# mlpc-ucsd/BDM

Measured on AMD Instinct MI355X. Metric: sampled shapes/sec (4096 pts, 1000 DDPM steps), higher is better.
Workload: dtype f32

## Files before the change

bdm_amd/csrc/pvconv_compact.hip:

```cpp
#include <stdlib.h>

#include "../../include/bdm_hip.h"
#include "common.h"
#include "gn_rule.h"
#include "h2_split.h"
#include "se_fc.h"
#include "trilinear.h"

using namespace bdm;

typedef __attribute__((ext_vector_type(8))) _Float16 f16x8;

namespace {

__device__ __forceinline__ void all_group_stats(const double *__restrict__ partial, int bi, int G, int S, double count, float eps,
                                                float *s_mean, float *s_rstd) {
  const int tid = threadIdx.x, l = tid & 31, gq = tid >> 5, per = blockDim.x >> 5;
  for (int g0 = 0; g0 < G; g0 += per) {
    const int g = g0 + gq;
    double a = 0.0, q = 0.0;
    if (g < G) {
      const double *pp = partial + ((size_t)bi * G + g) * S * 2;
      for (int sl = l; sl < S; sl += 32) { a += pp[2 * sl]; q += pp[2 * sl + 1]; }
    }
    a = half32_sum(a); q = half32_sum(q);
    if (l == 0 && g < G) gn_mean_rstd(a, q, count, eps, s_mean[g], s_rstd[g]);
  }
  __syncthreads();
}

}

__global__ __launch_bounds__(256) void to_h2_rows_kernel(int C, int V, int G, int S, int n_rows_max, int tiles_max, int dense_in,
                                                         const float *__restrict__ x, const int *__restrict__ dil_list,
                                                         const int *__restrict__ tile_start, const float *__restrict__ bias,
                                                         const double *__restrict__ partial, const float *__restrict__ gamma,
                                                         const float *__restrict__ beta, float eps, int act, float act_scale,
                                                         uint4 *__restrict__ rows_h2, uint4 *__restrict__ const_h2,
                                                         float *__restrict__ const_f32, unsigned *__restrict__ saturated) {
  __shared__ float s_mean[64], s_rstd[64];
  __shared__ float s_a[256], s_b[256];
  const int bi = blockIdx.y, tid = threadIdx.x, lane = tid & 63;
  const int C8 = (C + 7) / 8;
  const int nd = tile_start[((size_t)bi * tiles_max + tiles_max - 1) * 16 + 1];
  constexpr int RB = 512;
  if ((int)blockIdx.x * RB >= nd && blockIdx.x != 0) return;
  const int cg = C / G;
  const float g_pre = tid < C ? gamma[tid] : 0.f, b_pre = tid < C ? beta[tid] : 0.f;
  const int per_pass = blockDim.x / C8;
  const int c8 = tid % C8, rl = tid / C8;
  const int nch = min(8, C - c8 * 8);
  const bool vec = (C & 3) == 0 && nch == 8;
  auto load_row = [&](int j, float (&in)[8]) {
    if (dense_in) {
      const int v = dil_list[(size_t)bi * n_rows_max + j];
      const float *xb = x + ((size_t)bi * C + c8 * 8) * V + v;
#pragma unroll
      for (int u = 0; u < 8; ++u) in[u] = xb[(size_t)min(u, nch - 1) * V];
    } else {
      const float *row = x + ((size_t)bi * n_rows_max + j) * C + c8 * 8;
      if (vec) {
        const float4 p = *reinterpret_cast<const float4 *>(row), q = *reinterpret_cast<const float4 *>(row + 4);
        in[0] = p.x; in[1] = p.y; in[2] = p.z; in[3] = p.w; in[4] = q.x; in[5] = q.y; in[6] = q.z; in[7] = q.w;
      } else {
#pragma unroll
        for (int u = 0; u < 8; ++u) in[u] = row[min(u, nch - 1)];
      }
    }
  };
  const int j_end = min(nd, (int)(blockIdx.x + 1) * RB), j_first = blockIdx.x * RB + rl;
  const bool pre4 = rl < per_pass && j_first + 3 * per_pass < j_end;
  float pin0[8], pin1[8], pin2[8], pin3[8];
  if (pre4) { load_row(j_first, pin0); load_row(j_first + per_pass, pin1); load_row(j_first + 2 * per_pass, pin2); load_row(j_first + 3 * per_pass, pin3); }
  all_group_stats(partial, bi, G, S, (double)cg * V, eps, s_mean, s_rstd);
  for (int ch = tid; ch < C8 * 8; ch += blockDim.x) {
    float a = 0.f, bsh = 0.f;
    if (ch < C) {
      const int g = ch / cg;
      a = g_pre * s_rstd[g];
      bsh = b_pre - s_mean[g] * a;
    }
    s_a[ch] = a; s_b[ch] = bsh;
  }
  __syncthreads();
  bool sat = false;
  if (blockIdx.x == 0 && tid < C8) {
    const int c8 = tid, nch = min(8, C - c8 * 8);
    float fill[8];
#pragma unroll
    for (int j = 0; j < 8; ++j) {
      const int ch = c8 * 8 + j;
      float t = (ch < C && bias ? bias[ch] : 0.f) * s_a[ch] + s_b[ch];
      if (act == 1) t = swishf(t);
      fill[j] = ch < C ? t * act_scale : 0.f;
      sat |= !(fabsf(fill[j]) <= 65504.f);
    }
    uint4 ph, pl;
    split2_record(fill, ph, pl);
    const_h2[((size_t)bi * C8 + c8) * 2 + 0] = ph;
    const_h2[((size_t)bi * C8 + c8) * 2 + 1] = pl;
    const f16x8 hh = *reinterpret_cast<const f16x8 *>(&ph), ll = *reinterpret_cast<const f16x8 *>(&pl);
    for (int j = 0; j < nch; ++j) const_f32[(size_t)bi * C + c8 * 8 + j] = ((float)hh[j] + (float)ll[j]) * (1.0f / act_scale);
  }
  float ca[8], cb[8];
#pragma unroll
  for (int j = 0; j < 8; ++j) { ca[j] = s_a[c8 * 8 + j]; cb[j] = s_b[c8 * 8 + j]; }
  if (rl < per_pass) {
    auto emit_row = [&](int j, const float (&in)[8]) {
      float val[8];
#pragma unroll
      for (int u = 0; u < 8; ++u) {
        float t = in[u] * ca[u] + cb[u];
        if (act == 1) t = swishf(t);
        val[u] = t * act_scale;
        sat |= !(fabsf(val[u]) <= 65504.f);
      }
      uint4 ph, pl;
      split2_record(val, ph, pl);
      rows_h2[(((size_t)bi * C8 + c8) * 2 + 0) * n_rows_max + j] = ph;
      rows_h2[(((size_t)bi * C8 + c8) * 2 + 1) * n_rows_max + j] = pl;
    };
    int j = j_first;
    if (pre4) {
      emit_row(j, pin0); emit_row(j + per_pass, pin1); emit_row(j + 2 * per_pass, pin2); emit_row(j + 3 * per_pass, pin3);
      j += 4 * per_pass;
    }
    for (; j + 3 * per_pass < j_end; j += 4 * per_pass) {
      float in0[8], in1[8], in2[8], in3[8];
      load_row(j, in0); load_row(j + per_pass, in1); load_row(j + 2 * per_pass, in2); load_row(j + 3 * per_pass, in3);
      emit_row(j, in0); emit_row(j + per_pass, in1); emit_row(j + 2 * per_pass, in2); emit_row(j + 3 * per_pass, in3);
    }
    for (; j < j_end; j += per_pass) {
      float in0[8];
      load_row(j, in0);
      emit_row(j, in0);
    }
  }
  if (saturated != nullptr && __ballot(sat) != 0ull && lane == __ffsll((long long)__ballot(sat)) - 1) atomicOr(saturated, 1u);
}

extern "C" int bdm_group_norm_to_h2_rows(int b, int c, int v, int groups, const float *x, int dense_in, int n_rows_max,
                                         const int *dil_list, const int *tile_start, int tiles_max, const float *bias,
                                         const float *gamma, const float *beta, float eps, int act, float act_scale, void *rows_h2,
                                         void *const_h2, float *const_f32, const void *partial, int slices,
                                         unsigned int *saturated, void *stream) {
  BDM_REQUIRE(b >= 0 && c >= 1 && c <= 256 && v >= 1 && groups >= 1 && groups <= 64 && c % groups == 0 && (c / groups) >= 4 &&
                  partial != nullptr && slices >= 1 && x != nullptr && dil_list != nullptr && tile_start != nullptr && tiles_max >= 1 &&
                  n_rows_max >= 1 && rows_h2 && const_h2 && const_f32,
              "group_norm_to_h2_rows: bad arguments (<= 256 channels)");
  BDM_REQUIRE(h2_scale_is_pow2(act_scale), "group_norm_to_h2_rows: act_scale must be a power of two (got %g)", (double)act_scale);
  if (b == 0) return BDM_OK;
  dim3 grid(cdiv(n_rows_max, 512), b);
  hipLaunchKernelGGL(to_h2_rows_kernel, grid, dim3(256), 0, (hipStream_t)stream, c, v, groups, slices, n_rows_max, tiles_max, dense_in, x,
                     dil_list, tile_start, bias, (const double *)partial, gamma, beta, eps, act, act_scale, (uint4 *)rows_h2,
                     (uint4 *)const_h2, const_f32, saturated);
  return launch_status("group_norm_to_h2_rows");
}

__global__ void class_weight_sums_kernel(int cout, int cin, const float *__restrict__ w, double *__restrict__ wsum) {
  const long long total = 27ll * cin * cout;
  for (long long e = (long long)blockIdx.x * blockDim.x + threadIdx.x; e < total; e += (long long)gridDim.x * blockDim.x) {
    const int co = (int)(e % cout), ci = (int)((e / cout) % cin), k = (int)(e / ((long long)cout * cin));
    const int cls[3] = {k / 9, (k / 3) % 3, k % 3};
    double a = 0.0;
    for (int t = 0; t < 27; ++t) {
      const int d[3] = {t / 9 - 1, (t / 3) % 3 - 1, t % 3 - 1};
      bool in = true;
      for (int ax = 0; ax < 3; ++ax) in = in && !(cls[ax] == 0 && d[ax] == -1) && !(cls[ax] == 2 && d[ax] == 1);
      if (in) a += (double)w[((size_t)co * cin + ci) * 27 + t];
    }
    wsum[e] = a;
  }
}
extern "C" size_t bdm_conv3d_class_weight_elems(int cout, int cin) { return (size_t)27 * cin * cout; }
extern "C" int bdm_conv3d_class_weight_sums(int cout, int cin, const float *w, void *wsum, void *stream) {
  BDM_REQUIRE(cout >= 1 && cin >= 1 && w != nullptr && wsum != nullptr, "conv3d_class_weight_sums: bad arguments");
  hipLaunchKernelGGL(class_weight_sums_kernel, dim3(256), dim3(256), 0, (hipStream_t)stream, cout, cin, w, (double *)wsum);
  return launch_status("conv3d_class_weight_sums");
}

__global__ __launch_bounds__(256) void class_constants_kernel(int cin, int cout, const double *__restrict__ wsum, const float *__restrict__ bias,
                                                              const float *__restrict__ const_f32, const int *__restrict__ class_count,
                                                              float *__restrict__ class_vals, int G, int S, int slice0,
                                                              double *__restrict__ gn_partial) {
  __shared__ float s_c[256];
  __shared__ float s_v[256];
  const int k = blockIdx.x, bi = blockIdx.y, tid = threadIdx.x;
  for (int ci = tid; ci < cin; ci += blockDim.x) s_c[ci] = const_f32[(size_t)bi * cin + ci];
  __syncthreads();
  const double *wk = wsum + (size_t)k * cin * cout;
  for (int co = tid; co < cout; co += blockDim.x) {
    double a = bias ? (double)bias[co] : 0.0;
#pragma unroll 8
    for (int ci = 0; ci < cin; ++ci) a += wk[(size_t)ci * cout + co] * (double)s_c[ci];
    const float v = (float)a;
    class_vals[((size_t)bi * 27 + k) * cout + co] = v;
    s_v[co] = v;
  }
  __syncthreads();
  if (gn_partial != nullptr && tid < G) {
    const int cg = cout / G;
    double a = 0.0, q = 0.0;
    for (int j = 0; j < cg; ++j) { const double v = (double)s_v[tid * cg + j]; a += v; q += v * v; }
    const double n = (double)class_count[(size_t)bi * 27 + k];
    double *dst = gn_partial + (((size_t)bi * G + tid) * S + slice0 + k) * 2;
    dst[0] = n * a;
    dst[1] = n * q;
  }
}
extern "C" int bdm_conv3d_class_constants(int b, int cin, int cout, const void *wsum, const float *bias, const float *const_f32,
                                          const int *class_count, float *class_vals, int groups, void *gn_partial, int slices,
                                          int slice0, void *stream) {
  BDM_REQUIRE(b >= 0 && cin >= 1 && cin <= 256 && cout >= 1 && cout <= 256 && wsum && const_f32 && class_count && class_vals,
              "conv3d_class_constants: bad arguments (<= 256 channels)");
  BDM_REQUIRE(gn_partial == nullptr || (groups >= 1 && groups <= 64 && cout % groups == 0 && slice0 >= 0 && slice0 + 27 <= slices),
              "conv3d_class_constants: bad GroupNorm slice arguments");
  if (b == 0) return BDM_OK;
  hipLaunchKernelGGL(class_constants_kernel, dim3(27, b), dim3(256), 0, (hipStream_t)stream, cin, cout, (const double *)wsum, bias, const_f32,
                     class_count, class_vals, groups, slices, slice0, (double *)gn_partial);
  return launch_status("conv3d_class_constants");
}

#define SE_SLABS 64
struct GnFoldC {
  const double *partial;
  int S, G, l;
  const float *gamma, *beta;
  float eps;
};

__global__ __launch_bounds__(256) void se_rows_partial_kernel(int c, int V, int G, int S, int n_rows_max, int tiles_max,
                                                              const float *__restrict__ rows, const int *__restrict__ tile_start,
                                                              const double *__restrict__ partial, const float *__restrict__ gamma,
                                                              const float *__restrict__ beta, float eps, float2 *__restrict__ coef,
                                                              float *__restrict__ part, GnFoldC pf, float2 *__restrict__ pf_coef) {
  __shared__ float s_mean[64], s_rstd[64];
  __shared__ float s_a[256], s_b[256];
  __shared__ float s_acc[256];
  const int slab = blockIdx.x, bi = blockIdx.y, tid = threadIdx.x;
  const int cg = c / G;
  all_group_stats(partial, bi, G, S, (double)cg * V, eps, s_mean, s_rstd);
  for (int ch = tid; ch < c; ch += blockDim.x) {
    const float2 ab = gn_affine(gamma[ch], s_rstd[ch / cg], beta[ch], s_mean[ch / cg]);
    s_a[ch] = ab.x;
    s_b[ch] = ab.y;
  }
  __syncthreads();
  if (slab == 0) {
    for (int ch = tid; ch < c; ch += blockDim.x) coef[(size_t)bi * c + ch] = make_float2(s_a[ch], s_b[ch]);
    if (pf.partial != nullptr) {
      const int cgp = c / pf.G;
      for (int ch = tid; ch < c; ch += blockDim.x) {
        const int gp = ch / cgp;
        double a = 0.0, q = 0.0;
        const double *p = pf.partial + ((size_t)bi * pf.G + gp) * pf.S * 2;
        for (int s = 0; s < pf.S; ++s) { a += p[2 * s]; q += p[2 * s + 1]; }
        float mu, rstd;
        gn_mean_rstd(a, q, (double)cgp * pf.l, pf.eps, mu, rstd);
        pf_coef[(size_t)bi * c + ch] = gn_affine(pf.gamma[ch], rstd, pf.beta[ch], mu);
      }
    }
  }
  const int nd = tile_start[((size_t)bi * tiles_max + tiles_max - 1) * 16 + 1];
  const int per = (nd + SE_SLABS - 1) / SE_SLABS, j_lo = slab * per, j_hi = min(nd, j_lo + per);
  const int CL = c < 256 ? c : 256, RL = 256 / CL;
  const int cl = tid % CL, rl = tid / CL;
  for (int c0 = 0; c0 < c; c0 += CL) {
    const int ch = c0 + cl;
    float acc = 0.f;
    if (rl < RL && ch < c) {
      const float ga = s_a[ch], be = s_b[ch];
      const float *col = rows + (size_t)bi * n_rows_max * c + ch;
      float a0 = 0.f, a1 = 0.f, a2 = 0.f, a3 = 0.f;
      int j = j_lo + rl;
      for (; j + 7 * RL < j_hi; j += 8 * RL) {
        const float v0 = col[(size_t)j * c], v1 = col[(size_t)(j + RL) * c], v2 = col[(size_t)(j + 2 * RL) * c], v3 = col[(size_t)(j + 3 * RL) * c];
        const float v4 = col[(size_t)(j + 4 * RL) * c], v5 = col[(size_t)(j + 5 * RL) * c], v6 = col[(size_t)(j + 6 * RL) * c], v7 = col[(size_t)(j + 7 * RL) * c];
        a0 += swishf(v0 * ga + be); a1 += swishf(v1 * ga + be); a2 += swishf(v2 * ga + be); a3 += swishf(v3 * ga + be);
        a0 += swishf(v4 * ga + be); a1 += swishf(v5 * ga + be); a2 += swishf(v6 * ga + be); a3 += swishf(v7 * ga + be);
      }
      for (; j + 3 * RL < j_hi; j += 4 * RL) {
        const float v0 = col[(size_t)j * c], v1 = col[(size_t)(j + RL) * c], v2 = col[(size_t)(j + 2 * RL) * c], v3 = col[(size_t)(j + 3 * RL) * c];
        a0 += swishf(v0 * ga + be); a1 += swishf(v1 * ga + be); a2 += swishf(v2 * ga + be); a3 += swishf(v3 * ga + be);
      }
      for (; j < j_hi; j += RL) a0 += swishf(col[(size_t)j * c] * ga + be);
      acc = (a0 + a1) + (a2 + a3);
    }
    __syncthreads();
    s_acc[tid] = acc;
    __syncthreads();
    if (tid < CL && c0 + tid < c) {
      float a = 0.f;
      for (int r2 = 0; r2 < RL; ++r2) a += s_acc[r2 * CL + tid];
      part[((size_t)bi * SE_SLABS + slab) * c + c0 + tid] = a;
    }
  }
}

__global__ void se_rows_fc_kernel(int c, int h, int V, const float *__restrict__ part, const float2 *__restrict__ coef,
                                  const float *__restrict__ class_vals, const int *__restrict__ class_count,
                                  const float *__restrict__ w1, const float *__restrict__ w2, float *__restrict__ mean,
                                  float *__restrict__ gate) {
  extern __shared__ float sh[];
  float *s = sh, *hid = sh + c;
  const int bi = blockIdx.x;
  for (int i = threadIdx.x; i < c; i += blockDim.x) {
    double a = 0.0;
// ... 170 lines not shown
```

bdm_amd/modules.py:

```python
import os
from typing import NamedTuple

import torch
import torch.nn as nn

from . import functional as F
from . import ops
from . import tape

__all__ = ["Swish", "SharedMLP", "SE3d", "Voxelization", "Attention", "PVConv", "BallQuery",
           "PointNetSAModule", "PointNetFPModule"]


class Swish(nn.Module):

    def forward(self, x):
        raise RuntimeError("Swish is fused into bdm_group_norm on the HIP path")


class SharedMLP(nn.Module):

    def __init__(self, in_channels, out_channels, dim=1):
        super().__init__()
        if dim == 1:
# ... 197 lines not shown
        conv1, pconv = self.voxel_layers[0], self.point_features.layers[0]
        key = (conv1.weight._version, conv1.weight.data_ptr(), pconv.weight._version, pconv.weight.data_ptr(), c_t)
        hit = getattr(self, "_temb_rows", None)
        if hit is None or hit[0] != key:
            cout, c_feat = conv1.out_channels, self.in_channels - c_t
            wv = conv1.weight.detach()[:, c_feat:].reshape(cout, c_t, 27).permute(2, 0, 1).reshape(27 * cout, c_t)
            wp = pconv.weight.detach().reshape(pconv.out_channels, -1)[:, c_feat:]
            hit = (key, torch.cat([wv, wp], dim=0).contiguous())
            self._temb_rows = hit
        return hit[1]

    def can_split_temb(self, features, temb):
        B, c_feat, n = features.shape
        return (ops.is_point_invariant(temb) and not ops.is_point_invariant(features) and c_feat + temb.shape[1] == self.in_channels
                and self.route(B, n, cuda=features.is_cuda, temb_split=True, c_feat=c_feat).temb_split)

    def _temb_split_terms(self, features, temb):
        cout, B = self.voxel_layers[0].out_channels, features.shape[0]
        terms, self._temb_terms = self._temb_terms, None
        if terms is None or tuple(terms.shape) != (B, 28 * cout):
            tvec = temb[:, :, 0].contiguous()
            terms = ops.pointwise_conv(tvec[:, :, None], self.temb_rows(temb.shape[1]))[:, :, 0]
        return terms[:, :27 * cout], terms[:, 27 * cout:]

    se_in_devox = False
    fold_gn1 = True
    fold_pf = True
    point_stream = True
    point_stream_min = int(os.environ.get("BDM_POINT_STREAM_MIN", "8192"))
    _streams = {}

    compact_tail = os.environ.get("BDM_COMPACT_TAIL", "1")
    compact_tail_resolutions = {int(v) for v in os.environ.get("BDM_COMPACT_TAIL_R", "32,16").split(",") if v}

    _cond = None
    _next_pv = None

    def _parts(self):
        layers = list(self.voxel_layers)
        rest = [m for m in layers[2:] if isinstance(m, (nn.Conv3d, nn.GroupNorm, Attention, SE3d))]
        return (layers[0], layers[1], rest[0], rest[1], next((m for m in rest if isinstance(m, Attention)), None),
                next((m for m in rest if isinstance(m, SE3d)), None))

    def route(self, batch, n_points, *, cuda=True, hoisted=False, temb_split=False, c_feat=None, rows_offered=False):
        r = self.resolution
        conv1, gn1, conv2, gn2, att, se = self._parts()
        c1, c2 = conv1.out_channels, conv2.out_channels
        n_max = min(n_points, r ** 3)
        two_term = self.conv_impl in ("bf16x6", "fp16x3")
        h2 = self.conv_impl == "fp16x3" and not getattr(self, "h2_saturated", False)
        sparse = two_term and self.sparse_first_conv and r in self.sparse_resolutions
        dil = (sparse and self.sparse_conv == "dil" and r in self.sparse_dil_resolutions and h2 and self.sparse_gemm == "sparse_h2"
               and (self.sparse_dil_always or ops.sparse_dil_pays(batch, n_points, r, c1)))
        split = (temb_split and self.temb_split and cuda and sparse and not dil and c_feat is not None and c_feat % 8 == 0
                 and self.sparse_gemm in ("sparse_h2", "sparse_s3") and len(self.point_features.layers) == 3
                 and self.point_features.layers[0].out_channels == c1)
        cg2, tile = c2 // gn2.num_groups, (64 if (c2 > 32 and r != 8) else 32)
        folded = h2 and self.fold_gn2 and att is None and se is not None and cg2 in (4, 8, 16, 32) and tile % cg2 == 0

        impl, stats = None, False
        if not sparse:
            first = "dense_s3" if two_term else "dense_fp32"
        else:
            impl = self.sparse_gemm
            wide16 = n_max <= 1024 and (c_feat if split else conv1.in_channels) >= 128 and c1 >= 128
            if impl == "sparse_h2" and n_max > 256 and not wide16:
# ... 133 lines not shown
                impl = route.gemm_impl
                rows = rows_in if (route.takes_rows and rows_in.plan is plan and rows_in.channels == conv1.in_channels) else None
                if route.first == "gemm_split":
                    xh = ops.sparse_first_conv_planned(features, plan, self._packed_weight(conv1, impl), conv1.bias, cout, rows=rows, impl=impl,
                                                       h2_out=(gn1, ops.h2_activation_scale(gn1), ops.saturation_slot(self, features.device)))
                    return _VoxelBranch(None, None, plan, plan.norm_coords, xh)
                cin = features.shape[1] if col_bias is not None else None
                v = ops.sparse_first_conv_planned(features, plan, self._packed_weight(conv1, impl, cin=cin), conv1.bias, cout,
                                                  gn_groups=groups, rows=rows, col_bias=col_bias, impl=impl)
        return _VoxelBranch(*(v if groups else (v, None)), plan, plan.norm_coords)

    def _second_conv(self, route, vb):
        r = self.resolution
        _, gn1, conv2, gn2, _, _ = self._parts()
        cin, cout = conv2.in_channels, conv2.out_channels
        if route.second == "fp32":
            ops.group_norm_(vb.v, gn1.weight, gn1.bias, 8, gn1.eps, swish=True)
            vb.v = ops.conv3d(vb.v, self._packed_weight(conv2, "fp32"), conv2.bias, r)
        elif route.second == "bf16x6":
            vb.v = ops.conv3d_s3(ops.to_s3(vb.v, gn1, swish=True), self._packed_weight(conv2, "bf16x6"), conv2.bias, cin, cout, r)
        else:
            if vb.xh is None:
                sat = ops.saturation_slot(self, vb.v.device) if vb.v.is_cuda else None
                vb.xh = ops.to_h2(vb.v, gn1, swish=True, saturated=sat, stats=vb.gn1_stats)
            if route.tail == "plain":
                vb.v = ops.conv3d_h2(vb.xh, self._packed_weight(conv2, "fp16x3"), conv2.bias, cin, cout, r)
            else:
                vb.v, vb.stats = ops.conv3d_h2_gn(vb.xh, self._packed_weight(conv2, "fp16x3"), conv2.bias, cin, cout, r, gn2.num_groups)

    def _tail_lists(self, route, vb, pf, pf_ready, pf_pending):
        conv1, gn1, conv2, gn2, _, se = self._parts()
        plan, norm_coords = vb.plan, vb.norm_coords
        sat = ops.saturation_slot(self, pf.device)
        rows_h2, const_h2, const_f32, inv_s = ops.to_h2_rows(vb.v, plan, gn1, vb.gn1_stats, saturated=sat, bias=conv1.bias)
        y2, cvals, st2 = ops.second_conv_rows(rows_h2, const_h2, const_f32, inv_s, plan, self._packed_weight(conv2, "fp16x3"),
                                              self._packed_weight(conv2, "class"), conv2.bias, conv2.in_channels,
                                              conv2.out_channels, gn2.num_groups)
        w1, w2 = se.fc[0].weight, se.fc[2].weight
        if pf_pending is not None:
            if pf_ready is not None:
                tape.wait_event(pf_ready)
            gate, coef, pf_coef = ops.se_gate_gn_rows(y2, cvals, plan, st2, gn2, w1, w2, pf=pf_pending, n_points=pf.shape[2])
            return ops.devoxelize_gn_gate_add_rows(norm_coords, y2, cvals, plan, coef, gate=gate, add=pf, add_coef=pf_coef)
        gate, coef = ops.se_gate_gn_rows(y2, cvals, plan, st2, gn2, w1, w2)
        if pf_ready is not None:
            tape.wait_event(pf_ready)
        return ops.devoxelize_gn_gate_add_rows(norm_coords, y2, cvals, plan, coef, gate=gate, add=pf)

    def _tail_small(self, route, vb, pf, pf_ready, pf_pending):
        _, _, conv2, gn2, _, se = self._parts()
        head = None
        if route.head:
            head = vb.plan, ops.h2_sum_scale([gn2, self.point_features.layers[-2]]), ops.saturation_slot(self._next_pv, pf.device)
        if pf_ready is not None:
            tape.wait_event(pf_ready)
        pf_coef = None
        if pf_pending is not None:
            mean, coef, pf_coef = ops.se_means_gn(vb.v, vb.stats, gn2, pf=pf_pending, n_points=pf.shape[2])
        else:
            mean, coef = ops.se_means_gn(vb.v, vb.stats, gn2)
        out, rows = ops.pvconv_tail_small(vb.norm_coords, vb.v, coef, mean, se.fc[0].weight, se.fc[2].weight, self.resolution, add=pf, add_coef=pf_coef,
                                          head=head)
        if rows is not None:
            out._bdm_rows = rows
        return out

    def _tail_se_devox(self, route, vb, pf, pf_ready, pf_pending):
        _, _, _, gn2, _, se = self._parts()
        mean, coef = ops.se_means_gn(vb.v, vb.stats, gn2)
        if pf_ready is not None:
# ... 270 lines not shown
```

bdm_amd/ops.py:

```python
import ctypes
import math
import os
import warnings
import weakref

import torch

from . import _lib as L
from . import tape


def _bcl(t):
    if t.dtype != torch.float32:
        raise L.BdmHipError(f"expected float32, got {t.dtype}")
    B, C = t.shape[0], t.shape[1]
    if B * C > 0 and t.is_contiguous():
        l = t.numel() // (B * C)
        return t, B, C, l, C * l, l
    l = 1
    for s in t.shape[2:]:
        l *= s
    dense, exp = True, 1
    for d in range(t.dim() - 1, 1, -1):
        if t.shape[d] != 1 and t.stride(d) != exp:
# ... 1178 lines not shown
        for b in range(B):
            v = torch.nonzero(idx[b] >= 0).squeeze(1)
            out[b, :, v] = self.rows[b, idx[b, v]].t()
        return out


def sparse_first_conv_os(features, plan, packed, bias, cout, gn_groups=None, compact=False):
    plan_dilation(plan)
    if plan.dil_list is None:
        raise L.BdmHipError(f"sparse_first_conv_os: resolution {plan.r} has no dilated plan (8, 16, 32)")
    f, B, C, n, bs_f, ld_f = _bcl(features)
    dev, lib, r = f.device, L.lib(), plan.r
    packed_w, inv_scale = packed
    xr, slots = _records_f32((f, B, C, n, bs_f, ld_f), plan, extra=1)
    amax, counter = slots[:B], slots[B:]
    if compact:
        y = torch.empty(B, plan.n_dil_max, cout, dtype=torch.float32, device=dev)
        out = CompactGrid(y, plan, bias, cout)
    else:
        y = out = torch.empty(B, cout, r ** 3, dtype=torch.float32, device=dev)
    args = (B, C, cout, r, plan.n_max, plan.n_dil_max, L.ptr(xr), L.ptr(amax), L.ptr(plan.occ_index), L.ptr(plan.dil_list),
            L.ptr(plan.dil_index), L.ptr(plan.tile_start), L.ptr(packed_w), L.ptr(inv_scale), L.ptr(bias), L.ptr(y), 1 if compact else 0)
    if gn_groups:
        tiles = plan.tile_start.shape[1]
        partial = torch.empty(B, gn_groups, tiles, 2, dtype=torch.float64, device=dev)
        slices = ctypes.c_int(0)
        L.check(lib.bdm_sparse_conv_dil_gn(*args, int(gn_groups), L.ptr(partial), ctypes.byref(slices), plan.tile, L.ptr(counter), L.stream()),
                "sparse_conv_dil_gn")
        return out, (partial, tiles, int(gn_groups))
    L.check(lib.bdm_sparse_conv_dil(*args, plan.tile, L.ptr(counter), L.stream()), "sparse_conv_dil")
    return out


def to_h2_rows(x, plan, gn, stats, swish=True, saturated=None, bias=None):
    plan_dilation(plan)
    lib = L.lib()
    compact = isinstance(x, CompactGrid)
    src = x.rows if compact else x.contiguous()
    bias = x.bias if compact else bias
    B, C, V = src.shape[0], (x.channels if compact else src.shape[1]), plan.r ** 3
    dev = src.device
    s = float(h2_activation_scale(gn))
    C8 = (C + 7) // 8
    rows = torch.empty(B, C8, 2, plan.n_dil_max, 8, dtype=torch.float16, device=dev)
    const_h2 = torch.empty(B, C8, 2, 8, dtype=torch.float16, device=dev)
    const_f32 = torch.empty(B, C, dtype=torch.float32, device=dev)
    partial, slices, groups = stats
    L.check(lib.bdm_group_norm_to_h2_rows(B, C, V, groups, L.ptr(src), 0 if compact else 1, plan.n_dil_max, L.ptr(plan.dil_list),
                                          L.ptr(plan.tile_start), plan.tile_start.shape[1], L.ptr(bias), L.ptr(gn.weight), L.ptr(gn.bias),
                                          L.c_float(gn.eps), 1 if swish else 0, L.c_float(s), L.ptr(rows), L.ptr(const_h2), L.ptr(const_f32),
                                          L.ptr(partial), slices, L.ptr(saturated), L.stream()), "group_norm_to_h2_rows")
    return rows, const_h2, const_f32, 1.0 / s


def conv_class_pack(weight):
    cout, cin = weight.shape[:2]
    lib = L.lib()
    wsum = torch.empty(lib.bdm_conv3d_class_weight_elems(cout, cin), dtype=torch.float64, device=weight.device)
    L.check(lib.bdm_conv3d_class_weight_sums(cout, cin, L.ptr(weight.contiguous()), L.ptr(wsum), L.stream()), "conv3d_class_weight_sums")
    return wsum


def second_conv_rows(rows_h2, const_h2, const_f32, x_inv_scale, plan, packed, wsum, bias, cin, cout, groups=8):
    plan_dilation2(plan)
    lib, B, r = L.lib(), rows_h2.shape[0], plan.r
    dev = rows_h2.device
    packed_w, inv_scale = packed
    y = torch.empty(B, plan.n_dil_max, cout, dtype=torch.float32, device=dev)
    tiles = plan.d2_tiles.shape[1]
    partial = torch.empty(B, groups, tiles + 27, 2, dtype=torch.float64, device=dev)
    counter = amax_slots(dev, 1)
    slices = ctypes.c_int(0)
    L.check(lib.bdm_sparse_conv_dil_h2_gn(B, cin, cout, r, plan.n_dil_max, plan.n_dil_max, L.ptr(rows_h2), L.ptr(const_h2), L.c_float(x_inv_scale),
                                          L.ptr(plan.dil_index), L.ptr(plan.d2_list), L.ptr(plan.d2_index), L.ptr(plan.d2_tiles), L.ptr(packed_w),
                                          L.ptr(inv_scale), L.ptr(bias), L.ptr(y), int(groups), L.ptr(partial), ctypes.byref(slices), plan.d2_tile,
                                          L.ptr(counter), L.stream()), "sparse_conv_dil_h2_gn")
    assert slices.value == tiles + 27
    class_vals = torch.empty(B, 27, cout, dtype=torch.float32, device=dev)
    L.check(lib.bdm_conv3d_class_constants(B, cin, cout, L.ptr(wsum), L.ptr(bias), L.ptr(const_f32), L.ptr(plan.d2_class_count), L.ptr(class_vals),
                                           int(groups), L.ptr(partial), tiles + 27, tiles, L.stream()), "conv3d_class_constants")
    return y, class_vals, (partial, tiles + 27)


def se_gate_gn_rows(rows, class_vals, plan, stats, gn, w1, w2, pf=None, n_points=0):
    partial, slices = stats
    B, C = rows.shape[0], rows.shape[2]
    dev, lib = rows.device, L.lib()
    V = plan.r ** 3
    mean = torch.empty(B, C, dtype=torch.float32, device=dev)
    coef = torch.empty(B, C, 2, dtype=torch.float32, device=dev)
    gate = torch.empty(B, C, dtype=torch.float32, device=dev)
    part = torch.empty(lib.bdm_se_gate_gn_rows_workspace_elems(B, C), dtype=torch.float32, device=dev)
    args = (B, C, w1.shape[0], V, gn.num_groups, L.ptr(rows), plan.n_dil_max, L.ptr(plan.d2_tiles), plan.d2_tiles.shape[1], L.ptr(class_vals),
            L.ptr(plan.d2_class_count), L.ptr(partial), slices, L.ptr(gn.weight), L.ptr(gn.bias), L.c_float(gn.eps), L.ptr(w1), L.ptr(w2), L.ptr(part),
            L.ptr(mean), L.ptr(coef), L.ptr(gate))
    if pf is not None:
        (pp, ps, pg), pgn = pf
        pf_coef = torch.empty(B, C, 2, dtype=torch.float32, device=dev)
        L.check(lib.bdm_se_gate_gn_rows_pf(*args, L.ptr(pp), ps, pg, int(n_points), L.ptr(pgn.weight), L.ptr(pgn.bias), L.c_float(pgn.eps),
                                           L.ptr(pf_coef), L.stream()), "se_gate_gn_rows_pf")
        return gate, coef, pf_coef
    L.check(lib.bdm_se_gate_gn_rows(*args, L.stream()), "se_gate_gn_rows")
    return gate, coef


def devoxelize_gn_gate_add_rows(norm_coords, rows, class_vals, plan, coef, gate=None, add=None, add_coef=None):
    B, C = rows.shape[0], rows.shape[2]
    n = norm_coords.shape[2]
    out = torch.empty(B, C, n, dtype=torch.float32, device=rows.device)
    _, _, _, _, bs_o, ld_o = _bcl(out)
# ... 69 lines not shown
```

include/bdm_hip.h:

```cpp
#ifndef BDM_HIP_H
#define BDM_HIP_H

#include <stddef.h>
#include <stdint.h>

#ifdef __cplusplus
extern "C" {
#endif

const char *bdm_last_error(void);
int bdm_abi_version(void);


int bdm_furthest_point_sampling(int b, int n, int m, const float *coords, int *indices,
                                float *centers_out, void *stream);

int bdm_gather_features_forward(int b, int c, int n, int m, const float *features,
                                const int *indices, float *out, void *stream);

int bdm_ball_query(int b, int n, int m, float radius, int u, const float *centers,
                   const float *points, int *neighbors, void *stream);

int bdm_grouping_forward(int b, int c, int n, int m, int u, const float *features,
                         const int *indices, float *out, void *stream);
// ... 239 lines not shown
int bdm_sparse_conv_fused_pack_weights(int cout, int cin, const float *w, void *packed, float *scale_ws,
                                       float *inv_scale, void *stream);
int bdm_sparse_conv_fused(int b, int cin, int cout, int r, int n_max, const void *xr, const float *amax,
                          const void *packed_w, const float *inv_scale, const int *occ_list, const int *n_occ,
                          const float *bias, float *out, void *stream);
#endif

size_t bdm_sparse_conv_h2_weight_elems(int cout, int cin);
int bdm_sparse_conv_pack_weights_h2(int cout, int cin, const float *w, void *packed, float *scale_ws,
                                    float *inv_scale, void *stream);
int bdm_sparse_split_h2(int b, int cin, int n_max, const void *xr, const float *amax, void *xh, void *stream);
int bdm_sparse_conv_gemm_h2(int b, int n_max, int cin, int cout, const void *xh, const float *amax, const void *packed_w,
                            const float *inv_scale, const int *n_occ, float *y, void *stream);
int bdm_sparse_conv_gemm_h2_cb(int b, int n_max, int cin, int cout, const void *xh, const float *amax, const void *packed_w,
                               const float *inv_scale, const int *n_occ, const float *col_bias, long long bs_cb, float *y, void *stream);

int bdm_voxel_dilate_slices(int r, int tile);
int bdm_voxel_dilate(int b, int r, int n_dil_max, const int *cnt, int *dil_list, int *dil_index, int *plane_start, int *tile_start,
                     int tile, void *stream);
int bdm_sparse_conv_dil(int b, int cin, int cout, int r, int n_max, int n_dil_max, const void *xr, const float *amax,
                        const int *occ_index, const int *dil_list, const int *dil_index, const int *tile_start,
                        const void *packed_w, const float *inv_scale, const float *bias, float *y, int compact, int tile,
                        int *work_counter, void *stream);
int bdm_sparse_conv_dil_gn(int b, int cin, int cout, int r, int n_max, int n_dil_max, const void *xr, const float *amax,
                           const int *occ_index, const int *dil_list, const int *dil_index, const int *tile_start,
                           const void *packed_w, const float *inv_scale, const float *bias, float *y, int compact, int groups,
                           void *gn_partial, int *slices_out, int tile, int *work_counter, void *stream);

int bdm_voxel_dilate_again(int b, int r, int n_dil_max, const int *dil_index_in, int *dil_list, int *dil_index, int *plane_start,
                           int *tile_start, int *class_count, int tile, void *stream);
int bdm_group_norm_to_h2_rows(int b, int c, int v, int groups, const float *x, int dense_in, int n_rows_max, const int *dil_list,
                              const int *tile_start, int tiles_max, const float *bias, const float *gamma, const float *beta,
                              float eps, int act, float act_scale, void *rows_h2, void *const_h2, float *const_f32,
                              const void *partial, int slices, unsigned int *saturated, void *stream);
int bdm_sparse_conv_dil_h2_gn(int b, int cin, int cout, int r, int n_rows_max, int n_dil_max, const void *rows_h2, const void *xconst,
                              float x_inv_scale, const int *in_index, const int *dil_list, const int *dil_index,
                              const int *tile_start, const void *packed_w, const float *inv_scale, const float *bias, float *y,
                              int groups, void *gn_partial, int *slices_out, int tile, int *work_counter, void *stream);
size_t bdm_conv3d_class_weight_elems(int cout, int cin);
int bdm_conv3d_class_weight_sums(int cout, int cin, const float *w, void *wsum, void *stream);
int bdm_conv3d_class_constants(int b, int cin, int cout, const void *wsum, const float *bias, const float *const_f32,
                               const int *class_count, float *class_vals, int groups, void *gn_partial, int slices, int slice0,
                               void *stream);
size_t bdm_se_gate_gn_rows_workspace_elems(int b, int c);
int bdm_se_gate_gn_rows(int b, int c, int hidden, int v, int groups, const float *rows, int n_rows_max, const int *tile_start,
                        int tiles_max, const float *class_vals, const int *class_count, const void *gn_partial, int slices,
                        const float *gamma, const float *beta, float eps, const float *w1, const float *w2, float *part_ws,
                        float *mean_ws, float *coef, float *gate, void *stream);
int bdm_se_gate_gn_rows_pf(int b, int c, int hidden, int v, int groups, const float *rows, int n_rows_max, const int *tile_start,
                           int tiles_max, const float *class_vals, const int *class_count, const void *gn_partial, int slices,
                           const float *gamma, const float *beta, float eps, const float *w1, const float *w2, float *part_ws,
                           float *mean_ws, float *coef, float *gate, const void *pf_partial, int pf_slices, int pf_groups, int pf_n,
                           const float *pf_gamma, const float *pf_beta, float pf_eps, float *pf_coef, void *stream);
int bdm_devoxelize_gn_gate_add_rows(int b, int c, int n, int r, const float *coords, const float *rows, int n_rows_max,
                                    const int *dil_index, const float *class_vals, const float *coef, const float *gate,
                                    const float *add, long long bs_a, int ld_a, float *out, long long bs_o, int ld_o, void *stream);
int bdm_devoxelize_gn_gate_add_rows_pf(int b, int c, int n, int r, const float *coords, const float *rows, int n_rows_max,
                                       const int *dil_index, const float *class_vals, const float *coef, const float *gate,
                                       const float *add, long long bs_a, int ld_a, const float *add_coef, float *out, long long bs_o,
                                       int ld_o, void *stream);


int bdm_ddpm_step(long long n, const float *x, const float *eps, const float *noise,
                  float sqrt_beta_prod, float sqrt_alpha_prod, float coef_x0, float coef_x,
                  float sigma, float *out, void *stream);
int bdm_ddpm_step_dev(long long n, const float *x, const float *eps, const float *noise, const float *coef,
                      float *out, void *stream);
// ... 175 lines not shown
```

Measured before the change: 2.988.

## Fold class-constant computation into the h2 rows kernel and prefetch SE-gate rows

After: 2.998, median of 6. About the same (+0.3%).

```diff
diff --git a/bdm_amd/csrc/pvconv_compact.hip b/bdm_amd/csrc/pvconv_compact.hip
--- a/bdm_amd/csrc/pvconv_compact.hip
+++ b/bdm_amd/csrc/pvconv_compact.hip
@@ -29,22 +29,60 @@
   __syncthreads();
 }
 
-}
-
+__device__ __forceinline__ void class_constants_body(int k, int bi, int cin, int cout, const double *__restrict__ wsum,
+                                                     const float *__restrict__ bias, const int *__restrict__ class_count,
+                                                     float *__restrict__ class_vals, int G, int S, int slice0,
+                                                     double *__restrict__ gn_partial, const float *s_c, float *s_v) {
+  const int tid = threadIdx.x;
+  const double *wk = wsum + (size_t)k * cin * cout;
+  for (int co = tid; co < cout; co += blockDim.x) {
+    double a = bias ? (double)bias[co] : 0.0;
+#pragma unroll 8
+    for (int ci = 0; ci < cin; ++ci) a += wk[(size_t)ci * cout + co] * (double)s_c[ci];
+    const float v = (float)a;
+    class_vals[((size_t)bi * 27 + k) * cout + co] = v;
+    s_v[co] = v;
+  }
+  __syncthreads();
+  if (gn_partial != nullptr && tid < G) {
+    const int cg = cout / G;
+    double a = 0.0, q = 0.0;
+    for (int j = 0; j < cg; ++j) { const double v = (double)s_v[tid * cg + j]; a += v; q += v * v; }
+    const double n = (double)class_count[(size_t)bi * 27 + k];
+    double *dst = gn_partial + (((size_t)bi * G + tid) * S + slice0 + k) * 2;
+    dst[0] = n * a;
+    dst[1] = n * q;
+  }
+}
+
+struct ClassFold {
+  int cout, G, S, slice0;
+  const double *wsum;
+  const float *bias;
+  const int *class_count;
+  float *class_vals;
+  double *gn_partial;
+};
+
+}
+
+template <bool CC>
 __global__ __launch_bounds__(256) void to_h2_rows_kernel(int C, int V, int G, int S, int n_rows_max, int tiles_max, int dense_in,
                                                          const float *__restrict__ x, const int *__restrict__ dil_list,
                                                          const int *__restrict__ tile_start, const float *__restrict__ bias,
                                                          const double *__restrict__ partial, const float *__restrict__ gamma,
                                                          const float *__restrict__ beta, float eps, int act, float act_scale,
                                                          uint4 *__restrict__ rows_h2, uint4 *__restrict__ const_h2,
-                                                         float *__restrict__ const_f32, unsigned *__restrict__ saturated) {
+                                                         float *__restrict__ const_f32, unsigned *__restrict__ saturated,
+                                                         ClassFold cf) {
   __shared__ float s_mean[64], s_rstd[64];
   __shared__ float s_a[256], s_b[256];
   const int bi = blockIdx.y, tid = threadIdx.x, lane = tid & 63;
   const int C8 = (C + 7) / 8;
   const int nd = tile_start[((size_t)bi * tiles_max + tiles_max - 1) * 16 + 1];
   constexpr int RB = 512;
-  if ((int)blockIdx.x * RB >= nd && blockIdx.x != 0) return;
+  const int k_cls = CC ? (int)blockIdx.x - ((int)gridDim.x - 27) : -1;
+  if (k_cls < 0 && (int)blockIdx.x * RB >= nd && blockIdx.x != 0) return;
   const int cg = C / G;
   const float g_pre = tid < C ? gamma[tid] : 0.f, b_pre = tid < C ? beta[tid] : 0.f;
   const int per_pass = blockDim.x / C8;
@@ -69,7 +107,7 @@
     }
   };
   const int j_end = min(nd, (int)(blockIdx.x + 1) * RB), j_first = blockIdx.x * RB + rl;
-  const bool pre4 = rl < per_pass && j_first + 3 * per_pass < j_end;
+  const bool pre4 = k_cls < 0 && rl < per_pass && j_first + 3 * per_pass < j_end;
   float pin0[8], pin1[8], pin2[8], pin3[8];
   if (pre4) { load_row(j_first, pin0); load_row(j_first + per_pass, pin1); load_row(j_first + 2 * per_pass, pin2); load_row(j_first + 3 * per_pass, pin3); }
   all_group_stats(partial, bi, G, S, (double)cg * V, eps, s_mean, s_rstd);
@@ -84,8 +122,7 @@
   }
   __syncthreads();
   bool sat = false;
-  if (blockIdx.x == 0 && tid < C8) {
-    const int c8 = tid, nch = min(8, C - c8 * 8);
+  auto const_record = [&](int c8, uint4 &ph, uint4 &pl, float (&cf32)[8]) {
     float fill[8];
 #pragma unroll
     for (int j = 0; j < 8; ++j) {
@@ -95,12 +132,35 @@
       fill[j] = ch < C ? t * act_scale : 0.f;
       sat |= !(fabsf(fill[j]) <= 65504.f);
     }
+    split2_record(fill, ph, pl);
+    const f16x8 hh = *reinterpret_cast<const f16x8 *>(&ph), ll = *reinterpret_cast<const f16x8 *>(&pl);
+#pragma unroll
+    for (int j = 0; j < 8; ++j) cf32[j] = ((float)hh[j] + (float)ll[j]) * (1.0f / act_scale);
+  };
+  if constexpr (CC) {
+    if (k_cls >= 0) {
+      __shared__ float s_c[256], s_v[256];
+      if (tid < C8) {
+        uint4 ph, pl;
+        float cf32[8];
+        const_record(tid, ph, pl, cf32);
+        const int nch = min(8, C - tid * 8);
+        for (int j = 0; j < nch; ++j) s_c[tid * 8 + j] = cf32[j];
+      }
+      __syncthreads();
+      class_constants_body(k_cls, bi, C, cf.cout, cf.wsum, cf.bias, cf.class_count, cf.class_vals, cf.G, cf.S, cf.slice0, cf.gn_partial, s_c,
+                           s_v);
+      return;
+    }
+  }
+  if (blockIdx.x == 0 && tid < C8) {
+    const int c8 = tid, nch = min(8, C - c8 * 8);
     uint4 ph, pl;
-    split2_record(fill, ph, pl);
+    float cf32[8];
+    const_record(c8, ph, pl, cf32);
     const_h2[((size_t)bi * C8 + c8) * 2 + 0] = ph;
     const_h2[((size_t)bi * C8 + c8) * 2 + 1] = pl;
-    const f16x8 hh = *reinterpret_cast<const f16x8 *>(&ph), ll = *reinterpret_cast<const f16x8 *>(&pl);
-    for (int j = 0; j < nch; ++j) const_f32[(size_t)bi * C + c8 * 8 + j] = ((float)hh[j] + (float)ll[j]) * (1.0f / act_scale);
+    for (int j = 0; j < nch; ++j) const_f32[(size_t)bi * C + c8 * 8 + j] = cf32[j];
   }
   float ca[8], cb[8];
 #pragma unroll
@@ -143,17 +203,32 @@
                                          const int *dil_list, const int *tile_start, int tiles_max, const float *bias,
                                          const float *gamma, const float *beta, float eps, int act, float act_scale, void *rows_h2,
                                          void *const_h2, float *const_f32, const void *partial, int slices,
-                                         unsigned int *saturated, void *stream) {
+                                         unsigned int *saturated, int cout2, const void *wsum, const float *bias2,
+                                         const int *class_count, float *class_vals, int groups2, void *gn_partial2, int slices2,
+                                         int slice0, void *stream) {
   BDM_REQUIRE(b >= 0 && c >= 1 && c <= 256 && v >= 1 && groups >= 1 && groups <= 64 && c % groups == 0 && (c / groups) >= 4 &&
                   partial != nullptr && slices >= 1 && x != nullptr && dil_list != nullptr && tile_start != nullptr && tiles_max >= 1 &&
                   n_rows_max >= 1 && rows_h2 && const_h2 && const_f32,
               "group_norm_to_h2_rows: bad arguments (<= 256 channels)");
   BDM_REQUIRE(h2_scale_is_pow2(act_scale), "group_norm_to_h2_rows: act_scale must be a power of two (got %g)", (double)act_scale);
+  if (wsum != nullptr) {
+    BDM_REQUIRE(cout2 >= 1 && cout2 <= 256 && class_count && class_vals, "group_norm_to_h2_rows: bad class arguments (<= 256 channels)");
+    BDM_REQUIRE(gn_partial2 == nullptr || (groups2 >= 1 && groups2 <= 64 && cout2 % groups2 == 0 && slice0 >= 0 && slice0 + 27 <= slices2),
+                "group_norm_to_h2_rows: bad GroupNorm slice arguments of the class constants");
+  }
   if (b == 0) return BDM_OK;
+  if (wsum != nullptr) {
+    dim3 grid(cdiv(n_rows_max, 512) + 27, b);
+    const ClassFold cf{cout2, groups2, slices2, slice0, (const double *)wsum, bias2, class_count, class_vals, (double *)gn_partial2};
+    hipLaunchKernelGGL(to_h2_rows_kernel<true>, grid, dim3(256), 0, (hipStream_t)stream, c, v, groups, slices, n_rows_max, tiles_max, dense_in, x,
+                       dil_list, tile_start, bias, (const double *)partial, gamma, beta, eps, act, act_scale, (uint4 *)rows_h2,
+                       (uint4 *)const_h2, const_f32, saturated, cf);
+    return launch_status("group_norm_to_h2_rows (+ class constants)");
+  }
   dim3 grid(cdiv(n_rows_max, 512), b);
-  hipLaunchKernelGGL(to_h2_rows_kernel, grid, dim3(256), 0, (hipStream_t)stream, c, v, groups, slices, n_rows_max, tiles_max, dense_in, x,
+  hipLaunchKernelGGL(to_h2_rows_kernel<false>, grid, dim3(256), 0, (hipStream_t)stream, c, v, groups, slices, n_rows_max, tiles_max, dense_in, x,
                      dil_list, tile_start, bias, (const double *)partial, gamma, beta, eps, act, act_scale, (uint4 *)rows_h2,
-                     (uint4 *)const_h2, const_f32, saturated);
+                     (uint4 *)const_h2, const_f32, saturated, ClassFold{});
   return launch_status("group_norm_to_h2_rows");
 }
 
@@ -188,25 +263,7 @@
   const int k = blockIdx.x, bi = blockIdx.y, tid = threadIdx.x;
   for (int ci = tid; ci < cin; ci += blockDim.x) s_c[ci] = const_f32[(size_t)bi * cin + ci];
   __syncthreads();
-  const double *wk = wsum + (size_t)k * cin * cout;
-  for (int co = tid; co < cout; co += blockDim.x) {
-    double a = bias ? (double)bias[co] : 0.0;
-#pragma unroll 8
-    for (int ci = 0; ci < cin; ++ci) a += wk[(size_t)ci * cout + co] * (double)s_c[ci];
-    const float v = (float)a;
-    class_vals[((size_t)bi * 27 + k) * cout + co] = v;
-    s_v[co] = v;
-  }
-  __syncthreads();
-  if (gn_partial != nullptr && tid < G) {
-    const int cg = cout / G;
-    double a = 0.0, q = 0.0;
-    for (int j = 0; j < cg; ++j) { const double v = (double)s_v[tid * cg + j]; a += v; q += v * v; }
-    const double n = (double)class_count[(size_t)bi * 27 + k];
-    double *dst = gn_partial + (((size_t)bi * G + tid) * S + slice0 + k) * 2;
-    dst[0] = n * a;
-    dst[1] = n * q;
-  }
+  class_constants_body(k, bi, cin, cout, wsum, bias, class_count, class_vals, G, S, slice0, gn_partial, s_c, s_v);
 }
 extern "C" int bdm_conv3d_class_constants(int b, int cin, int cout, const void *wsum, const float *bias, const float *const_f32,
                                           const int *class_count, float *class_vals, int groups, void *gn_partial, int slices,
@@ -239,9 +296,22 @@
   __shared__ float s_acc[256];
   const int slab = blockIdx.x, bi = blockIdx.y, tid = threadIdx.x;
   const int cg = c / G;
+  const float g_pre = tid < c ? gamma[tid] : 0.f, b_pre = tid < c ? beta[tid] : 0.f;
+  const int nd = tile_start[((size_t)bi * tiles_max + tiles_max - 1) * 16 + 1];
+  const int per = (nd + SE_SLABS - 1) / SE_SLABS, j_lo = slab * per, j_hi = min(nd, j_lo + per);
+  const int CL = c < 256 ? c : 256, RL = 256 / CL;
+  const int cl = tid % CL, rl = tid / CL;
+  const bool pre8 = rl < RL && cl < c && j_lo + rl + 7 * RL < j_hi;
+  float p0 = 0.f, p1 = 0.f, p2 = 0.f, p3 = 0.f, p4 = 0.f, p5 = 0.f, p6 = 0.f, p7 = 0.f;
+  if (pre8) {
+    const float *col = rows + (size_t)bi * n_rows_max * c + cl;
+    const int j = j_lo + rl;
+    p0 = col[(size_t)j * c]; p1 = col[(size_t)(j + RL) * c]; p2 = col[(size_t)(j + 2 * RL) * c]; p3 = col[(size_t)(j + 3 * RL) * c];
+    p4 = col[(size_t)(j + 4 * RL) * c]; p5 = col[(size_t)(j + 5 * RL) * c]; p6 = col[(size_t)(j + 6 * RL) * c]; p7 = col[(size_t)(j + 7 * RL) * c];
+  }
   all_group_stats(partial, bi, G, S, (double)cg * V, eps, s_mean, s_rstd);
   for (int ch = tid; ch < c; ch += blockDim.x) {
-    const float2 ab = gn_affine(gamma[ch], s_rstd[ch / cg], beta[ch], s_mean[ch / cg]);
+    const float2 ab = gn_affine(g_pre, s_rstd[ch / cg], b_pre, s_mean[ch / cg]);
     s_a[ch] = ab.x;
     s_b[ch] = ab.y;
   }
@@ -261,10 +331,6 @@
       }
     }
   }
-  const int nd = tile_start[((size_t)bi * tiles_max + tiles_max - 1) * 16 + 1];
-  const int per = (nd + SE_SLABS - 1) / SE_SLABS, j_lo = slab * per, j_hi = min(nd, j_lo + per);
-  const int CL = c < 256 ? c : 256, RL = 256 / CL;
-  const int cl = tid % CL, rl = tid / CL;
   for (int c0 = 0; c0 < c; c0 += CL) {
     const int ch = c0 + cl;
     float acc = 0.f;
@@ -273,6 +339,11 @@
       const float *col = rows + (size_t)bi * n_rows_max * c + ch;
       float a0 = 0.f, a1 = 0.f, a2 = 0.f, a3 = 0.f;
       int j = j_lo + rl;
+      if (c0 == 0 && pre8) {
+        a0 += swishf(p0 * ga + be); a1 += swishf(p1 * ga + be); a2 += swishf(p2 * ga + be); a3 += swishf(p3 * ga + be);
+        a0 += swishf(p4 * ga + be); a1 += swishf(p5 * ga + be); a2 += swishf(p6 * ga + be); a3 += swishf(p7 * ga + be);
+        j += 8 * RL;
+      }
       for (; j + 7 * RL < j_hi; j += 8 * RL) {
         const float v0 = col[(size_t)j * c], v1 = col[(size_t)(j + RL) * c], v2 = col[(size_t)(j + 2 * RL) * c], v3 = col[(size_t)(j + 3 * RL) * c];
         const float v4 = col[(size_t)(j + 4 * RL) * c], v5 = col[(size_t)(j + 5 * RL) * c], v6 = col[(size_t)(j + 6 * RL) * c], v7 = col[(size_t)(j + 7 * RL) * c];
diff --git a/bdm_amd/modules.py b/bdm_amd/modules.py
--- a/bdm_amd/modules.py
+++ b/bdm_amd/modules.py
@@ -253,6 +253,7 @@
 
     compact_tail = os.environ.get("BDM_COMPACT_TAIL", "1")
     compact_tail_resolutions = {int(v) for v in os.environ.get("BDM_COMPACT_TAIL_R", "32,16").split(",") if v}
+    compact_tail_fused = os.environ.get("BDM_COMPACT_TAIL_FUSED", "1") == "1"
 
     _cond = None
     _next_pv = None
@@ -452,10 +453,14 @@
         conv1, gn1, conv2, gn2, _, se = self._parts()
         plan, norm_coords = vb.plan, vb.norm_coords
         sat = ops.saturation_slot(self, pf.device)
-        rows_h2, const_h2, const_f32, inv_s = ops.to_h2_rows(vb.v, plan, gn1, vb.gn1_stats, saturated=sat, bias=conv1.bias)
-        y2, cvals, st2 = ops.second_conv_rows(rows_h2, const_h2, const_f32, inv_s, plan, self._packed_weight(conv2, "fp16x3"),
-                                              self._packed_weight(conv2, "class"), conv2.bias, conv2.in_channels,
-                                              conv2.out_channels, gn2.num_groups)
+        wsum, classes = self._packed_weight(conv2, "class"), None
+        if self.compact_tail_fused:
+            rows_h2, const_h2, const_f32, inv_s, classes = ops.to_h2_rows(vb.v, plan, gn1, vb.gn1_stats, saturated=sat, bias=conv1.bias,
+                                                                          classes=(wsum, conv2.bias, conv2.out_channels, gn2.num_groups))
+        else:
+            rows_h2, const_h2, const_f32, inv_s = ops.to_h2_rows(vb.v, plan, gn1, vb.gn1_stats, saturated=sat, bias=conv1.bias)
+        y2, cvals, st2 = ops.second_conv_rows(rows_h2, const_h2, const_f32, inv_s, plan, self._packed_weight(conv2, "fp16x3"), wsum,
+                                              conv2.bias, conv2.in_channels, conv2.out_channels, gn2.num_groups, classes=classes)
         w1, w2 = se.fc[0].weight, se.fc[2].weight
         if pf_pending is not None:
             if pf_ready is not None:
diff --git a/bdm_amd/ops.py b/bdm_amd/ops.py
--- a/bdm_amd/ops.py
+++ b/bdm_amd/ops.py
@@ -1234,7 +1234,7 @@
     return out
 
 
-def to_h2_rows(x, plan, gn, stats, swish=True, saturated=None, bias=None):
+def to_h2_rows(x, plan, gn, stats, swish=True, saturated=None, bias=None, classes=None):
     plan_dilation(plan)
     lib = L.lib()
     compact = isinstance(x, CompactGrid)
@@ -1248,10 +1248,19 @@
     const_h2 = torch.empty(B, C8, 2, 8, dtype=torch.float16, device=dev)
     const_f32 = torch.empty(B, C, dtype=torch.float32, device=dev)
     partial, slices, groups = stats
-    L.check(lib.bdm_group_norm_to_h2_rows(B, C, V, groups, L.ptr(src), 0 if compact else 1, plan.n_dil_max, L.ptr(plan.dil_list),
-                                          L.ptr(plan.tile_start), plan.tile_start.shape[1], L.ptr(bias), L.ptr(gn.weight), L.ptr(gn.bias),
-                                          L.c_float(gn.eps), 1 if swish else 0, L.c_float(s), L.ptr(rows), L.ptr(const_h2), L.ptr(const_f32),
-                                          L.ptr(partial), slices, L.ptr(saturated), L.stream()), "group_norm_to_h2_rows")
+    args = (B, C, V, groups, L.ptr(src), 0 if compact else 1, plan.n_dil_max, L.ptr(plan.dil_list), L.ptr(plan.tile_start),
+            plan.tile_start.shape[1], L.ptr(bias), L.ptr(gn.weight), L.ptr(gn.bias), L.c_float(gn.eps), 1 if swish else 0, L.c_float(s),
+            L.ptr(rows), L.ptr(const_h2), L.ptr(const_f32), L.ptr(partial), slices, L.ptr(saturated))
+    if classes is not None:
+        wsum, bias2, cout2, groups2 = classes
+        plan_dilation2(plan)
+        tiles = plan.d2_tiles.shape[1]
+        partial2 = torch.empty(B, groups2, tiles + 27, 2, dtype=torch.float64, device=dev)
+        class_vals = torch.empty(B, 27, cout2, dtype=torch.float32, device=dev)
+        L.check(lib.bdm_group_norm_to_h2_rows(*args, cout2, L.ptr(wsum), L.ptr(bias2), L.ptr(plan.d2_class_count), L.ptr(class_vals),
+                                              int(groups2), L.ptr(partial2), tiles + 27, tiles, L.stream()), "group_norm_to_h2_rows")
+        return rows, const_h2, const_f32, 1.0 / s, (class_vals, partial2)
+    L.check(lib.bdm_group_norm_to_h2_rows(*args, 0, None, None, None, None, 0, None, 0, 0, L.stream()), "group_norm_to_h2_rows")
     return rows, const_h2, const_f32, 1.0 / s
 
 
@@ -1263,14 +1272,18 @@
     return wsum
 
 
-def second_conv_rows(rows_h2, const_h2, const_f32, x_inv_scale, plan, packed, wsum, bias, cin, cout, groups=8):
+def second_conv_rows(rows_h2, const_h2, const_f32, x_inv_scale, plan, packed, wsum, bias, cin, cout, groups=8, classes=None):
     plan_dilation2(plan)
     lib, B, r = L.lib(), rows_h2.shape[0], plan.r
     dev = rows_h2.device
     packed_w, inv_scale = packed
     y = torch.empty(B, plan.n_dil_max, cout, dtype=torch.float32, device=dev)
     tiles = plan.d2_tiles.shape[1]
-    partial = torch.empty(B, groups, tiles + 27, 2, dtype=torch.float64, device=dev)
+    if classes is not None:
+        class_vals, partial = classes
+        assert tuple(partial.shape) == (B, groups, tiles + 27, 2) and tuple(class_vals.shape) == (B, 27, cout)
+    else:
+        partial = torch.empty(B, groups, tiles + 27, 2, dtype=torch.float64, device=dev)
     counter = amax_slots(dev, 1)
     slices = ctypes.c_int(0)
     L.check(lib.bdm_sparse_conv_dil_h2_gn(B, cin, cout, r, plan.n_dil_max, plan.n_dil_max, L.ptr(rows_h2), L.ptr(const_h2), L.c_float(x_inv_scale),
@@ -1278,6 +1291,8 @@
                                           L.ptr(inv_scale), L.ptr(bias), L.ptr(y), int(groups), L.ptr(partial), ctypes.byref(slices), plan.d2_tile,
                                           L.ptr(counter), L.stream()), "sparse_conv_dil_h2_gn")
     assert slices.value == tiles + 27
+    if classes is not None:
+        return y, class_vals, (partial, tiles + 27)
     class_vals = torch.empty(B, 27, cout, dtype=torch.float32, device=dev)
     L.check(lib.bdm_conv3d_class_constants(B, cin, cout, L.ptr(wsum), L.ptr(bias), L.ptr(const_f32), L.ptr(plan.d2_class_count), L.ptr(class_vals),
                                            int(groups), L.ptr(partial), tiles + 27, tiles, L.stream()), "conv3d_class_constants")
diff --git a/include/bdm_hip.h b/include/bdm_hip.h
--- a/include/bdm_hip.h
+++ b/include/bdm_hip.h
@@ -295,7 +295,9 @@
 int bdm_group_norm_to_h2_rows(int b, int c, int v, int groups, const float *x, int dense_in, int n_rows_max, const int *dil_list,
                               const int *tile_start, int tiles_max, const float *bias, const float *gamma, const float *beta,
                               float eps, int act, float act_scale, void *rows_h2, void *const_h2, float *const_f32,
-                              const void *partial, int slices, unsigned int *saturated, void *stream);
+                              const void *partial, int slices, unsigned int *saturated, int cout2, const void *wsum,
+                              const float *bias2, const int *class_count, float *class_vals, int groups2, void *gn_partial2,
+                              int slices2, int slice0, void *stream);
 int bdm_sparse_conv_dil_h2_gn(int b, int cin, int cout, int r, int n_rows_max, int n_dil_max, const void *rows_h2, const void *xconst,
                               float x_inv_scale, const int *in_index, const int *dil_list, const int *dil_index,
                               const int *tile_start, const void *packed_w, const float *inv_scale, const float *bias, float *y,
```
